# Daniel-Liu-c0deb0t/block-aligner

Hardware: AMD Instinct MI355X
Metric: GCUPS (DP cells/s) on 10 kbp DNA X-drop batch; bit-exact score+CIGAR vs AVX2 (higher is better)
Workload: dtype i16 (saturating lane scores) + i32 block offsets

## Files before the change

block_aligner_amd/csrc/ba_driver.hpp:

```cpp
#pragma once
#include "ba_device.hpp"

namespace ba {

#ifndef BA_BIG
#define BA_BIG 0
#endif
constexpr bool kBig = BA_BIG != 0;
__device__ __forceinline__ void lds_sync() {
    if (kBig) __builtin_amdgcn_fence(__ATOMIC_ACQ_REL, "workgroup");
    else __builtin_amdgcn_fence(__ATOMIC_ACQ_REL, "wavefront");
    __builtin_amdgcn_wave_barrier();
}
__device__ __forceinline__ void lds_fill0(short* a, uint32_t n) {
    for (uint32_t k = 2 * lane_id(); k < n; k += 128) *(int*)(a + k) = 0;
    lds_sync();
}
__device__ __forceinline__ void lds_copy(short* dst, const short* src, uint32_t n) {
    lds_sync();
    for (uint32_t k = 2 * lane_id(); k < n; k += 128) {
        const int v = *(const int*)(src + k);
        lds_sync();
        *(int*)(dst + k) = v;
    }
    lds_sync();
}
__device__ __forceinline__ int lds_prefix_max8(const short* a) {
    lds_sync();
    const int* p = (const int*)a;
    const s16x2 m = as_s(vmax(vmax(p[0], p[1]), vmax(p[2], p[3])));
    return uni(max((int)m.x, (int)m.y));
}
__device__ __forceinline__ int lds_suffix_max2(const short* a, uint32_t n) {
    lds_sync();
    s16x2 m = as_s(*(const int*)(a + n - 2));
    return uni(max((int)m.x, (int)m.y));
}
__device__ __forceinline__ int lds_shift_and_offset(uint32_t n, short* b1, short* b2, const short* t1, const short* t2, int off_add) {
    const int oa = splat(off_add);
    lds_sync();
    const int corner = uni((int)as_s(adds(splat((int)b1[STEP - 1]), oa)).x);
    for (uint32_t base = 0; base < n; base += 128) {
        const uint32_t k = base + 2 * lane_id();
        int v1 = 0, v2 = 0;
        const bool in = k < n;
        if (in) {
            if (k + STEP < n) {
                v1 = adds(*(const int*)(b1 + k + STEP), oa);
                v2 = adds(*(const int*)(b2 + k + STEP), oa);
            } else {
                v1 = *(const int*)(t1 + (k + STEP - n));
                v2 = *(const int*)(t2 + (k + STEP - n));
            }
        }
        lds_sync();
        if (in) { *(int*)(b1 + k) = v1; *(int*)(b2 + k) = v2; }
        lds_sync();
    }
    return corner;
}

struct Move { uint32_t op, di, dj, next; };
constexpr uint32_t TB_PENDING = 3;
__device__ __forceinline__ Move tb_lut(bool right_blk, uint32_t t, uint32_t t2, uint32_t table) {
    constexpr uint32_t OP_M = 1, OP_I = 4, OP_D = 5;
    const uint32_t gapA_op = right_blk ? OP_D : OP_I, gapB_op = right_blk ? OP_I : OP_D;
    const uint32_t A_di = right_blk ? 0 : 1, A_dj = right_blk ? 1 : 0;
    const uint32_t A_tab = right_blk ? 1 : 2, B_tab = right_blk ? 2 : 1;
    if (table == A_tab) return (t2 & 1) ? Move{gapA_op, A_di, A_dj, 0} : Move{gapA_op, A_di, A_dj, A_tab};
    if (table == B_tab) return Move{gapB_op, 1 - A_di, 1 - A_dj, TB_PENDING};
    if (t == 0) return Move{OP_M, 1, 1, 0};
    if (t & 1) return (t2 & 1) ? Move{gapA_op, A_di, A_dj, 0} : Move{gapA_op, A_di, A_dj, A_tab};
    return Move{gapB_op, 1 - A_di, 1 - A_dj, TB_PENDING};
}
__device__ __forceinline__ uint32_t tb_resolve(bool right_blk, uint32_t table, uint32_t nib) {
    return table == TB_PENDING ? ((nib & 8u) ? 0u : (right_blk ? 2u : 1u)) : table;
}
__device__ __forceinline__ uint32_t tb_next(bool right_blk, uint32_t next, uint32_t v) {
    return (next == TB_PENDING && v == 0) ? (right_blk ? 2u : 1u) : next;
}

template <bool RO>
__host__ __device__ constexpr uint32_t slot_cell_byte(uint32_t c) { return RO ? (((c & 2u) << 1) | ((c & 4u) >> 1) | (c & 1u)) : c; }

template <bool RO = false>
__device__ __forceinline__ uint32_t traceback(const BlockRec* __restrict__ blocks, uint32_t nblocks, const uint32_t* __restrict__ trace,
                                     uint32_t i, uint32_t j, const uint8_t* __restrict__ q, const uint8_t* __restrict__ r, uint32_t flags,
                                     uint32_t* __restrict__ out, uint64_t out_lo, uint64_t out_hi, uint32_t* status) {
    const bool eq = flags & F_CIGAR_EQ, local = flags & F_LOCAL, fqs = flags & F_FQS;
    bool stop = false;
    uint64_t wp = out_hi;
    uint32_t run_op = 0, run_len = 0;
    uint32_t table = 0;
    uint32_t bidx = nblocks;
    while ((i > 0 || j > 0) && !stop) {
        BlockRec br;
        for (;;) {
            if (bidx == 0) { *status |= ST_TRACEBACK_LOST; return 0; }
            bidx--;
            br = blocks[bidx];
            if (i >= (br.i & 0x7fffffffu) && j >= br.j) break;
        }
        const bool right_blk = br.trace_base >> 31;
        const bool l2 = br.i >> 31;
        br.i &= 0x7fffffffu;
        if (br.trace_base & 0x40000000u) { *status |= ST_TRACEBACK_LOST; return 0; }
        const uint32_t tbase = br.trace_base & 0x3fffffffu;
        const uint32_t Hv = right_blk ? br.h : br.w;
        const uint32_t nch = Hv > 128 ? Hv / 128 : 1, nl = Hv > 128 ? 64 : Hv / 2;
        while (i >= br.i && j >= br.j && (i > 0 || j > 0)) {
            const uint32_t ci = i - br.i, cj = j - br.j;
            const uint32_t v = right_blk ? ci : cj, w = right_blk ? cj : ci;
            const uint32_t chunk = v >> 7, lane = (v & 127) >> 1;
            if (right_blk && fqs && i == 0) { stop = true; break; }
            uint32_t nib;
            if (l2) {
                const uint32_t cb = slot_cell_byte<RO>(v & 7u);
                const uint32_t word = trace[tbase + (v >> 3) * 8 + (w >> 1) * 2 + (cb >> 2)];
                nib = ((word >> ((cb & 3) * 8 + (w & 1) * 4)) ^ 15u) & 15u;
            } else {
                const uint32_t word = trace[tbase + (((w >> 2) * nch + chunk) * nl + lane) * (local ? 2u : 1u)];
                nib = ((word >> ((v & 1) * 16 + (w & 3) * 4)) ^ 15u) & 15u;
            }
            table = tb_resolve(right_blk, table, nib);
            if (local && table == 0) {
                if (l2) {
                    const uint32_t z = trace[tbase + (uint32_t)br.h * br.w / 8 + (v >> 3) * 2 + ((v >> 2) & 1)];
                    if ((z >> ((v & 3) * 8 + w)) & 1) { stop = true; break; }
                } else {
                    const uint32_t z = trace[tbase + (((w >> 2) * nch + chunk) * nl + lane) * 2u + 1u];
                    if ((z >> ((v & 1) * 16 + (w & 3) * 4)) & 1) { stop = true; break; }
                }
            }
            const Move m = tb_lut(right_blk, nib & 3, (nib >> 2) & 1, table);
            uint32_t op = m.op;
            if (eq && op == 1) op = q[i] == r[j] ? 2 : 3;
            if (m.di > i || m.dj > j) { *status |= ST_TRACEBACK_LOST; return 0; }
            i -= m.di; j -= m.dj; table = tb_next(right_blk, m.next, v);
            if (op == run_op) run_len++;
            else {
                if (run_len) {
                    if (wp == out_lo) { *status |= ST_CIGAR_OVERFLOW; return 0; }
                    out[--wp] = (run_len << 4) | run_op;
                }
                run_op = op; run_len = 1;
            }
        }
    }
    if (run_len) {
        if (wp == out_lo) { *status |= ST_CIGAR_OVERFLOW; return 0; }
        out[--wp] = (run_len << 4) | run_op;
    }
    return (uint32_t)(out_hi - wp);
}

__device__ __forceinline__ uint32_t wave_excl_sum(uint32_t x, uint32_t lane) {
    uint32_t s = x;
#pragma unroll
    for (int d = 1; d < 64; d <<= 1) {
        const uint32_t o = (uint32_t)__shfl_up((int)s, d, 64);
        s += lane >= (uint32_t)d ? o : 0u;
    }
    return s - x;
}
template <bool L2OK, bool RO = false>
__device__ __forceinline__ uint32_t walk_wave(const BlockRec* __restrict__ blocks, uint32_t nblocks_in, const uint32_t* __restrict__ trace,
                                              uint32_t i_in, uint32_t j_in, const uint8_t* __restrict__ q, const uint8_t* __restrict__ r, bool eq,
                                              uint32_t* __restrict__ out, uint64_t out_lo, uint64_t out_hi, uint32_t* status,
                                              uint32_t* __restrict__ lds, uint32_t budget) {
    const uint32_t lane = (uint32_t)lane_id();
    uint32_t lutv0, lutv1;
    {
        const Move a = tb_lut(false, lane & 3, (lane >> 2) & 1, (lane >> 4) & 3), b = tb_lut(true, lane & 3, (lane >> 2) & 1, (lane >> 4) & 3);
        lutv0 = a.op | (a.di << 3) | (a.dj << 4) | (a.next << 5);
        lutv1 = b.op | (b.di << 3) | (b.dj << 4) | (b.next << 5);
    }
    uint32_t i = (uint32_t)uni((int)i_in), j = (uint32_t)uni((int)j_in), bidx = (uint32_t)uni((int)nblocks_in);
    uint32_t table = 0, run_op = 0, run_len = 0, nrun = 0, runbuf = 0, st = 0;
    uint64_t wp = out_hi;
    uint32_t qw0 = 0, rw0 = 0, qwin = 0, rwin = 0;
    auto load_q = [&]() { qw0 = i >= 252u ? (i - 252u) & ~3u : 0u; const uint32_t a = qw0 + 4u * lane; qwin = a <= i ? *(const uint32_t*)(q + a) : 0u; };
    auto load_r = [&]() { rw0 = j >= 252u ? (j - 252u) & ~3u : 0u; const uint32_t a = rw0 + 4u * lane; rwin = a <= j ? *(const uint32_t*)(r + a) : 0u; };
    if (eq) { load_q(); load_r(); }
    auto flush = [&]() {
        if (lane < nrun) out[wp - 1u - lane] = runbuf;
        wp -= nrun; nrun = 0;
    };
    auto emit = [&]() -> bool {
        if (!run_len) return true;
        if (wp - nrun == out_lo) return false;
        asm volatile("s_mov_b32 m0, %2\n\tv_writelane_b32 %0, %1, m0" : "+v"(runbuf) : "s"(__builtin_amdgcn_readfirstlane((int)((run_len << 4) | run_op))), "s"(__builtin_amdgcn_readfirstlane((int)nrun)) : "m0");
        if (++nrun == 64u) flush();
        return true;
    };
    bool ok = true;
    while (ok && (i > 0 || j > 0)) {
        if (bidx == 0) { st = ST_TRACEBACK_LOST; ok = false; break; }
        const uint32_t nvalid = min(bidx, 64u);
        uint4 rec = uint4{0, 0, 0, 0};
        if (lane < nvalid) rec = *(const uint4*)(blocks + (bidx - 1u - lane));
        const bool untr = rec.w & 0x40000000u;
        const uint32_t words = untr ? 0u : (rec.z & 0xffffu) * (rec.z >> 16) / 8u;
        const uint32_t tb = rec.w & 0x3fffffffu;
        uint32_t toff = wave_excl_sum(lane < nvalid ? words : 0u, lane);
        const uint32_t nfit = (uint32_t)__popcll(__ballot(lane < nvalid && toff + words <= budget));
        const uint32_t tb_up = (uint32_t)__shfl_up((int)tb, 1, 64);
        const bool flat = nfit > 1 && !__any(lane > 0 && lane < nfit && tb + words != tb_up);
        if (nfit > 0) {
            const uint32_t total = (uint32_t)__builtin_amdgcn_readlane((int)(toff + words), (int)(nfit - 1u));
            if (flat) {
                const uint32_t lo = (uint32_t)__builtin_amdgcn_readlane((int)tb, (int)(nfit - 1u));
                for (uint32_t x = lane; x < total; x += 64u) lds[x] = trace[lo + x];
                toff = tb - lo;
            } else {
                for (uint32_t k = 0; k < nfit; k++) {
                    const uint32_t base = (uint32_t)__builtin_amdgcn_readlane((int)tb, (int)k), sz = (uint32_t)__builtin_amdgcn_readlane((int)words, (int)k);
                    const uint32_t off = (uint32_t)__builtin_amdgcn_readlane((int)toff, (int)k);
                    for (uint32_t x = lane; x < sz; x += 64u) lds[off + x] = trace[base + x];
                }
            }
            asm volatile("s_waitcnt vmcnt(0) lgkmcnt(0)" ::: "memory");
        }
        const bool direct = nfit == 0;
        const uint32_t ntake = direct ? 1u : nfit;
        auto walk_rects = [&](auto direct_c) {
        constexpr bool DIRECT = decltype(direct_c)::value;
        uint32_t cur = 0;
        while (cur < ntake && ok && (i > 0 || j > 0)) {
            const uint32_t rx = (uint32_t)__builtin_amdgcn_readlane((int)rec.x, (int)cur), bj = (uint32_t)__builtin_amdgcn_readlane((int)rec.y, (int)cur);
            const uint32_t bi = rx & 0x7fffffffu;
            if (!(i >= bi && j >= bj)) { cur++; continue; }
            const uint32_t rz = (uint32_t)__builtin_amdgcn_readlane((int)rec.z, (int)cur), rw = (uint32_t)__builtin_amdgcn_readlane((int)rec.w, (int)cur);
            if (rw & 0x40000000u) { st = ST_TRACEBACK_LOST; ok = false; break; }
            const uint32_t off = DIRECT ? (rw & 0x3fffffffu) : (uint32_t)__builtin_amdgcn_readlane((int)toff, (int)cur);
            const bool right = rw >> 31, l2 = L2OK && (rx >> 31);
            const uint32_t Hv = right ? (rz & 0xffffu) : (rz >> 16);
            const uint32_t nch = Hv > 128u ? Hv / 128u : 1u, nl = Hv > 128u ? 64u : Hv / 2u;
            const uint32_t lutr = right ? lutv1 : lutv0;
            while (i >= bi && j >= bj && (i > 0 || j > 0)) {
                const uint32_t ci = i - bi, cj = j - bj;
                const uint32_t v = right ? ci : cj, w = right ? cj : ci;
                uint32_t widx, sh;
                if (l2) { const uint32_t cb = slot_cell_byte<RO>(v & 7u); widx = (v >> 3) * 8u + (w >> 1) * 2u + (cb >> 2); sh = (cb & 3u) * 8u + (w & 1u) * 4u; }
                else { widx = ((w >> 2) * nch + (v >> 7)) * nl + ((v & 127u) >> 1); sh = (v & 1u) * 16u + (w & 3u) * 4u; }
                uint32_t word;
                if (table == 0u && i > 0u && j > 0u && min(v, w) >= 1u) {
                    const uint32_t lim = min(min(v, w), min(i, j) - 1u);
                    const bool valid = lane <= lim;
                    const uint32_t vv = v - lane, ww = w - lane;
                    uint32_t widx_k, sh_k;
                    if (l2) { const uint32_t cb = slot_cell_byte<RO>(vv & 7u); widx_k = (vv >> 3) * 8u + (ww >> 1) * 2u + (cb >> 2); sh_k = (cb & 3u) * 8u + (ww & 1u) * 4u; }
                    else { widx_k = ((ww >> 2) * nch + (vv >> 7)) * nl + ((vv & 127u) >> 1); sh_k = (vv & 1u) * 16u + (ww & 3u) * 4u; }
                    uint32_t word_k = 0;
                    if (valid) { if constexpr (DIRECT) word_k = trace[off + widx_k]; else word_k = lds[off + widx_k]; }
                    const unsigned long long cm = __ballot(valid && ((word_k >> sh_k) & 3u) == 3u);
                    uint32_t n = cm == ~0ull ? 64u : (uint32_t)__builtin_ctzll(~cm);
                    if (eq && n >= 2u) {
                        if (i < qw0) load_q();
                        if (j < rw0) load_r();
                        n = min(n, min(i - qw0, j - rw0) + 1u);
                    }
                    if (n >= 2u) {
                        bool fits = true;
                        if (!eq) {
                            if (run_op == 1u) run_len += n;
                            else { fits = emit(); run_op = 1u; run_len = n; }
                        } else {
                            const uint32_t qa = i - lane - qw0, ra = j - lane - rw0;
                            const uint32_t qd = (uint32_t)__builtin_amdgcn_ds_bpermute((int)(qa & ~3u), (int)qwin), rd = (uint32_t)__builtin_amdgcn_ds_bpermute((int)(ra & ~3u), (int)rwin);
                            const bool same = ((qd >> ((qa & 3u) * 8u)) & 255u) == ((rd >> ((ra & 3u) * 8u)) & 255u);
                            unsigned long long bits = __ballot(lane < n && same);
                            uint32_t rem = n;
                            while (rem && fits) {
                                const bool e = bits & 1ull;
                                const unsigned long long x = e ? ~bits : bits;
                                const uint32_t len = min(x ? (uint32_t)__builtin_ctzll(x) : 64u, rem), op2 = e ? 2u : 3u;
                                if (op2 == run_op) run_len += len;
                                else { fits = emit(); run_op = op2; run_len = len; }
                                bits = len < 64u ? bits >> len : 0ull; rem -= len;
                            }
                        }
                        if (!fits) { st = ST_CIGAR_OVERFLOW; ok = false; break; }
                        i -= n; j -= n;
                        continue;
                    }
                    word = (uint32_t)__builtin_amdgcn_readlane((int)word_k, 0);
                } else {
                if constexpr (DIRECT) word = (uint32_t)uni((int)trace[off + widx]); else word = (uint32_t)uni((int)lds[off + widx]);
                }
                const uint32_t nib = ((word >> sh) ^ 15u) & 15u;
                table = tb_resolve(right, table, nib);
                const uint32_t m = (uint32_t)__builtin_amdgcn_readlane((int)lutr, (int)((table << 4) | nib));
                uint32_t op = m & 7u;
                const uint32_t di = (m >> 3) & 1u, dj = (m >> 4) & 1u;
                if (eq && op == 1u) {
                    if (i < qw0) load_q();
                    if (j < rw0) load_r();
                    const uint32_t qd = (uint32_t)__builtin_amdgcn_readlane((int)qwin, (int)((i - qw0) >> 2)), rd = (uint32_t)__builtin_amdgcn_readlane((int)rwin, (int)((j - rw0) >> 2));
                    op = ((qd >> ((i & 3u) * 8u)) & 255u) == ((rd >> ((j & 3u) * 8u)) & 255u) ? 2u : 3u;
                }
                if (di > i || dj > j) { st = ST_TRACEBACK_LOST; ok = false; break; }
                i -= di; j -= dj; table = tb_next(right, m >> 5, v);
                if (op == run_op) run_len++;
                else {
                    if (!emit()) { st = ST_CIGAR_OVERFLOW; ok = false; break; }
                    run_op = op; run_len = 1;
                }
            }
        }
        };
        if (direct) walk_rects(std::true_type{}); else walk_rects(std::false_type{});
        bidx -= ntake;
    }
    if (ok && !emit()) { st = ST_CIGAR_OVERFLOW; ok = false; }
    if (!ok) { *status |= st; return 0; }
    flush();
    return (uint32_t)(out_hi - wp);
}

#define BA_RLX_AGENT __ATOMIC_RELAXED, __HIP_MEMORY_SCOPE_AGENT

struct TbLane {
    uint32_t slot, pair, i, j, table, bidx, run_op, run_len, status;
    uint64_t wp, lo;
    const BlockRec* blocks; const uint32_t* trace; const uint8_t* q; const uint8_t* r;
    uint32_t bi, bj, tbase, zoff, nch, nl; bool right, in_rect, l2;
    uint4 nrec[4]; uint32_t nq;
    uint32_t tw_chunk, tw_g, tw_lane0; bool tw_ok;
    uint32_t qw0, rw0;
    uint32_t pv[6], po[6], pmask;
};

__device__ __forceinline__ void tb_emit(TbLane& t, uint32_t* __restrict__ out) {
    if (t.run_len) {
        if (t.wp == t.lo) { t.status |= ST_CIGAR_OVERFLOW; t.i = t.j = 0; return; }
        out[--t.wp] = (t.run_len << 4) | t.run_op;
    }
}
__device__ __forceinline__ void tb_fail(TbLane& t) { t.status |= ST_TRACEBACK_LOST; t.i = t.j = 0; t.run_len = 0; }

constexpr int TB_CELLS_PER_STEP = 4;
#ifndef BA_WALK_CELLS
#define BA_WALK_CELLS 8
#endif
#ifndef BA_RING_DEPTH
#define BA_RING_DEPTH 2
#endif
#ifndef BA_WALK_DEPTH
#define BA_WALK_DEPTH 4
#endif
#ifndef BA_HELPER_CELLS
#define BA_HELPER_CELLS 4
#endif
template <int CELLS = TB_CELLS_PER_STEP, int DEPTH = 1, int LB = (int)TB_LANE_BYTES, bool RO = false>
__device__ __forceinline__ void tb_step(TbLane& t, uint32_t flags, uint32_t* __restrict__ out, unsigned char* lrec,
                                        const unsigned char* lut, unsigned long long* tacc = nullptr) {
    constexpr bool LOCREC = LB == (int)TB_LANE_BYTES_LOC;
    constexpr bool L2OK = LB == (int)TB_LANE_BYTES_L2 || LOCREC;
    constexpr int SEQ_Q = LOCREC ? 80 : (L2OK ? 64 : 40), SEQ_R = SEQ_Q + 16;
    const bool eq = flags & F_CIGAR_EQ, local = LOCREC && (flags & F_LOCAL), fqs = flags & F_FQS;
    BA_TSTAMP(ts0);
    if (!t.in_rect || !(t.i >= t.bi && t.j >= t.bj)) {
        bool found = false, untraced = false;
#pragma unroll
        for (int a = 0; a < DEPTH; a++) {
            if (!found && (a == 0 || t.nq)) {
                if (t.bidx == 0) { tb_fail(t); return; }
                uint4 rec;
                if (t.nq) {
                    rec = t.nrec[0];
#pragma unroll
                    for (int k = 0; k + 1 < DEPTH; k++) t.nrec[k] = t.nrec[k + 1];
                    t.nq--;
                } else rec = *(const uint4*)(t.blocks + t.bidx - 1);
                t.bidx--;
                t.l2 = L2OK && (rec.x >> 31); t.bi = rec.x & 0x7fffffffu; t.bj = rec.y;
                const uint32_t h = rec.z & 0xffffu, w = rec.z >> 16;
                t.in_rect = t.i >= t.bi && t.j >= t.bj;
                t.zoff = h * w / 8;
                t.right = rec.w >> 31;
                t.tbase = rec.w & 0x3fffffffu;
                const uint32_t Hv = t.right ? h : w;
                t.nch = Hv > 128 ? Hv / 128 : 1; t.nl = Hv > 128 ? 64 : Hv / 2;
                untraced = rec.w & 0x40000000u;
                found = t.in_rect;
            }
        }
        if (t.nq == 0 && t.bidx > 0) {
#pragma unroll
            for (int k = 0; k < DEPTH; k++) if (t.bidx > (uint32_t)k) t.nrec[k] = *(const uint4*)(t.blocks + t.bidx - 1 - k);
            t.nq = min((uint32_t)DEPTH, t.bidx);
        }
        t.tw_ok = false;
        if (!t.in_rect) return;
        if (untraced) { tb_fail(t); return; }
    }
    {
        const uint32_t ci = t.i - t.bi, cj = t.j - t.bj;
        const uint32_t v = t.right ? ci : cj, w = t.right ? cj : ci;
        const uint32_t chunk = v >> 7, lc = (v & 127) >> 1, g = w >> 2;
        if (L2OK && t.l2) {
            const uint32_t L8 = v >> 3;
            if (!(t.tw_ok && t.tw_chunk == 0xffffu && L8 - t.tw_lane0 < 2u)) {
                t.tw_chunk = 0xffffu; t.tw_g = 0; t.tw_lane0 = L8 ? L8 - 1 : 0u; t.tw_ok = true;
                const uint32_t* wp = t.trace + t.tbase + t.tw_lane0 * 8;
                uint4 a0, a1, a2, a3;
                __builtin_memcpy(&a0, wp, 16); __builtin_memcpy(&a1, wp + 4, 16); __builtin_memcpy(&a2, wp + 8, 16); __builtin_memcpy(&a3, wp + 12, 16);
                uint4* lw = (uint4*)lrec;
                lw[0] = a0; lw[1] = a1; lw[2] = a2; lw[3] = a3;
                if (local) {
                    uint4 z;
                    __builtin_memcpy(&z, t.trace + t.tbase + t.zoff + t.tw_lane0 * 2, 16);
                    lw[4] = z;
                }
            }
        } else
        if (local) {
            if (!(t.tw_ok && chunk == t.tw_chunk && t.tw_g - g < 2u && lc - t.tw_lane0 < 5u)) {
                t.tw_chunk = chunk; t.tw_g = g; t.tw_lane0 = min(lc >= 4 ? lc - 4 : 0u, t.nl - 5u); t.tw_ok = true;
                const uint32_t* hi = t.trace + t.tbase + ((g * t.nch + chunk) * t.nl + t.tw_lane0) * 2u;
                const uint32_t* lo = g ? hi - t.nch * t.nl * 2u : hi;
                uint4 h0, h1, l0, l1; uint2 h2, l2;
                __builtin_memcpy(&h0, hi, 16); __builtin_memcpy(&h1, hi + 4, 16); __builtin_memcpy(&h2, hi + 8, 8);
                __builtin_memcpy(&l0, lo, 16); __builtin_memcpy(&l1, lo + 4, 16); __builtin_memcpy(&l2, lo + 8, 8);
                uint32_t* lw = (uint32_t*)lrec;
                lw[0] = h0.x; lw[1] = h0.y; lw[2] = h0.z; lw[3] = h0.w; lw[4] = h1.x; lw[5] = h1.y; lw[6] = h1.z; lw[7] = h1.w; lw[8] = h2.x; lw[9] = h2.y;
                lw[10] = l0.x; lw[11] = l0.y; lw[12] = l0.z; lw[13] = l0.w; lw[14] = l1.x; lw[15] = l1.y; lw[16] = l1.z; lw[17] = l1.w; lw[18] = l2.x; lw[19] = l2.y;
            }
        } else
        if (!(t.tw_ok && chunk == t.tw_chunk && t.tw_g - g < 2u && lc - t.tw_lane0 < 5u)) {
            t.tw_chunk = chunk; t.tw_g = g; t.tw_lane0 = min(lc >= 4 ? lc - 4 : 0u, t.nl - 5u); t.tw_ok = true;
            const uint32_t* hi = t.trace + t.tbase + (g * t.nch + chunk) * t.nl + t.tw_lane0;
            const uint32_t* lo = g ? hi - t.nch * t.nl : hi;
            uint32_t wv[10];
            {
                uint4 h4, l4;
                __builtin_memcpy(&h4, hi, 16); __builtin_memcpy(&l4, lo, 16);
                wv[0] = h4.x; wv[1] = h4.y; wv[2] = h4.z; wv[3] = h4.w; wv[4] = hi[4];
                wv[5] = l4.x; wv[6] = l4.y; wv[7] = l4.z; wv[8] = l4.w; wv[9] = lo[4];
            }
#pragma unroll
            for (int k = 0; k < 10; k++) ((uint32_t*)lrec)[k] = wv[k];
        }
        if (eq) {
            if (t.qw0 == 0xffffffffu || t.i < t.qw0 + 8 || t.i >= t.qw0 + 16) {
                t.qw0 = t.i >= 12 ? (t.i - 12) & ~3u : 0;
                const uint32_t* p = (const uint32_t*)(t.q + t.qw0);
                uint32_t b4[4];
#pragma unroll
                for (int k = 0; k < 4; k++) b4[k] = p[k];
#pragma unroll
                for (int k = 0; k < 4; k++) ((uint32_t*)lrec)[SEQ_Q / 4 + k] = b4[k];
            }
            if (t.rw0 == 0xffffffffu || t.j < t.rw0 + 8 || t.j >= t.rw0 + 16) {
                t.rw0 = t.j >= 12 ? (t.j - 12) & ~3u : 0;
                const uint32_t* p = (const uint32_t*)(t.r + t.rw0);
                uint32_t b4[4];
#pragma unroll
                for (int k = 0; k < 4; k++) b4[k] = p[k];
#pragma unroll
                for (int k = 0; k < 4; k++) ((uint32_t*)lrec)[SEQ_R / 4 + k] = b4[k];
            }
        }
    }
#ifdef BA_TIMING
    const unsigned long long ts1 = __builtin_amdgcn_s_memtime();
    asm volatile("s_waitcnt vmcnt(0)" ::: "memory");
    const unsigned long long ts2 = __builtin_amdgcn_s_memtime();
    if (tacc) { tacc[0] += ts1 - ts0; tacc[1] += ts2 - ts1; }
#endif
    {
        bool alive = true;
#pragma unroll
        for (int s = 0; s < CELLS; s++) {
            alive = alive && (t.i > 0 || t.j > 0) && t.i >= t.bi && t.j >= t.bj;
            const uint32_t ci = t.i - t.bi, cj = t.j - t.bj;
            const uint32_t v = t.right ? ci : cj, w = t.right ? cj : ci;
            const uint32_t lc = (v & 127) >> 1;
            if (fqs) {
                const bool stop = alive && t.right && t.i == 0;
                if (stop) t.i = t.j = 0;
                alive = alive && !stop;
            }
            const uint32_t gi = t.tw_g - (w >> 2);
            uint32_t baddr, zaddr = 0, zbit = 0;
            if (L2OK && t.l2) {
                const uint32_t k8 = (v >> 3) - t.tw_lane0;
                alive = alive && t.tw_chunk == 0xffffu && k8 <= 1u;
                baddr = k8 * 32 + (w >> 1) * 8 + slot_cell_byte<RO>(v & 7u);
                zaddr = 64 + k8 * 8 + ((v >> 2) & 1) * 4 + (v & 3); zbit = w;
            } else {
                const uint32_t k = lc - t.tw_lane0;
                alive = alive && (v >> 7) == t.tw_chunk && gi <= 1u && k <= 4u;
                baddr = local ? gi * 40 + k * 8 + (v & 1) * 2 + ((w & 3) >> 1) : gi * 20 + k * 4 + (v & 1) * 2 + ((w & 3) >> 1);
                zaddr = baddr + 4; zbit = (w & 1) * 4;
            }
            const uint32_t qo = t.i - t.qw0, ro = t.j - t.rw0;
            const uint32_t byte = lrec[alive ? baddr : 0u];
            const uint32_t qb = lrec[SEQ_Q + (qo & 15u)], rb = lrec[SEQ_R + (ro & 15u)];
            const uint32_t nib = ((byte >> ((w & 1) * 4)) ^ 15u) & 15u;
            const uint32_t table = tb_resolve(t.right, t.table, nib);
            if (local) {
                const uint32_t zb = lrec[alive ? zaddr : 0u];
                const bool stop = alive && table == 0 && ((zb >> zbit) & 1u);
                if (stop) t.i = t.j = 0;
                alive = alive && !stop;
            }
            const uint32_t m = lut[((uint32_t)t.right << 6) | (table << 4) | nib];
            uint32_t op = m & 7u;
            const uint32_t di = (m >> 3) & 1u, dj = (m >> 4) & 1u;
            const bool is_match = eq && op == 1;
            alive = alive && !(is_match && (qo > 15u || ro > 15u));
            if (is_match) op = qb == rb ? 2u : 3u;
            if (alive && (di > t.i || dj > t.j)) { tb_fail(t); alive = false; }
            const bool same = op == t.run_op;
            if (alive && !same && t.run_len) {
                if (t.wp == t.lo) { t.status |= ST_CIGAR_OVERFLOW; t.i = t.j = 0; alive = false; }
                else out[--t.wp] = (t.run_len << 4) | t.run_op;
            }
            t.i -= alive ? di : 0u; t.j -= alive ? dj : 0u;
            t.table = alive ? tb_next(t.right, m >> 5, v) : t.table;
            t.run_len = alive ? (same ? t.run_len + 1 : 1u) : t.run_len;
            t.run_op = alive ? op : t.run_op;
        }
    }
}

#ifndef BA_TB_FAST
#define BA_TB_FAST 1
#endif
#ifndef BA_TB_FCELLS
#define BA_TB_FCELLS 1
#endif
#ifndef BA_TB_DIAG_RUNS
#define BA_TB_DIAG_RUNS 2
#endif
#ifndef BA_TB_DIAG2
#define BA_TB_DIAG2 1
#endif
#ifndef BA_TB_FDEPTH
#define BA_TB_FDEPTH 3
#endif
typedef uint32_t tb_u32x4 __attribute__((ext_vector_type(4)));
__device__ __forceinline__ uint4 tb_ld16(const void* p) {
    typedef tb_u32x4 __attribute__((aligned(4))) V;
    const tb_u32x4 v = *(const V*)p;
    return uint4{v.x, v.y, v.z, v.w};
}
__device__ __forceinline__ uint32_t ffbl_u32(uint32_t x) { uint32_t r; asm("v_ffbl_b32 %0, %1" : "=v"(r) : "v"(x)); return r; }
__device__ __forceinline__ void tb_prefetch2(TbLane& t) {
    if (t.bidx > 0u) t.nrec[0] = *(const uint4*)(t.blocks + t.bidx - 1);
    if (t.bidx > 1u) t.nrec[1] = *(const uint4*)(t.blocks + t.bidx - 2);
    t.nq = min(2u, t.bidx);
}
template <bool L2W, bool RO = false>
__device__ __forceinline__ void tb_diag_lut_fill(unsigned char* dlut) {
    if constexpr (L2W) {
#pragma unroll
        for (int e = 0; e < 3; e++) {
            const uint32_t idx = (uint32_t)lane_id() + 64u * e;
            const uint32_t k = idx & 7u, p = idx >> 3;
            const uint32_t x = (p - k) & 15u, c = ((p - 16u) - k) & 7u;
            dlut[idx] = (unsigned char)(p < 16u ? (((x & 8u) << 2) | slot_cell_byte<RO>(x & 7u)) : ((c >> 1) << 3));
        }
    }
    {
        const uint32_t idx = (uint32_t)lane_id(), k = idx & 7u, x = ((idx >> 3) - k) & 7u;
        dlut[(L2W ? TB_DIAG_LUT_L2 - TB_DIAG_LUT_STD : 0u) + idx] = (unsigned char)((x < 4u ? 20u : 0u) + ((x & 3u) >> 1));
    }
}
template <int S>
__device__ __forceinline__ void tb_push(TbLane& t, const bool cond, const uint32_t val, bool& ovf) {
    const bool room = t.wp != t.lo, go = cond && room;
    t.wp -= go ? 1u : 0u;
    t.pv[S] = go ? val : t.pv[S];
    t.po[S] = go ? (uint32_t)t.wp - (uint32_t)t.lo : t.po[S];
    t.pmask |= go ? (1u << S) : 0u;
    ovf = ovf || (cond && !room);
}
__device__ __forceinline__ void tb_flush(TbLane& t, uint32_t* __restrict__ out) {
#pragma unroll
    for (int s = 0; s < 6; s++) if ((t.pmask >> s) & 1u) out[t.lo + t.po[s]] = t.pv[s];
    t.pmask = 0;
}

template <bool L2W, int SEQ_Q, int SEQ_R, int S0>
__device__ __forceinline__ void tb_diag(TbLane& t, const bool eq, const unsigned char* lrec, const unsigned char* dlut, bool& ovf) {
    static_assert(BA_TB_DIAG_RUNS >= 1 && BA_TB_DIAG_RUNS <= 2, "two slots per call site");
    const uint32_t ci = t.i - t.bi, cj = t.j - t.bj;
    const uint32_t v = t.right ? ci : cj, w = t.right ? cj : ci;
    bool ok = t.in_rect && t.tw_ok && t.i >= t.bi && t.j >= t.bj && (t.table == 0u || t.table == TB_PENDING);
    uint32_t K = min(min(t.i, t.j), min(v, w) + 1u);
// ... 1461 lines not shown
```

Baseline: 2700.

## Extend traceback diagonal run detection across staged block boundaries and skip redundant probes

In the LDS-staged traceback path, the wave-wide diagonal-match probe can now follow the diagonal across several staged blocks. It builds a per-diagonal-offset owner table in a reserved 64-word LDS slice and uses bpermute to fetch each lane's block record, so a run can jump directly to the block where it ends. A skip counter also suppresses re-probing after a known non-diagonal cell. This is meant to cut the number of serial probe iterations per traceback, at the cost of more per-probe work (prefix max, LDS writes, five bpermutes) and a slightly smaller staging budget.

```diff
diff --git a/block_aligner_amd/csrc/ba_driver.hpp b/block_aligner_amd/csrc/ba_driver.hpp
--- a/block_aligner_amd/csrc/ba_driver.hpp
+++ b/block_aligner_amd/csrc/ba_driver.hpp
@@ -169,6 +169,8 @@
                                               uint32_t* __restrict__ out, uint64_t out_lo, uint64_t out_hi, uint32_t* status,
                                               uint32_t* __restrict__ lds, uint32_t budget) {
     const uint32_t lane = (uint32_t)lane_id();
+    const uint32_t tbudget = budget - 64u;
+    uint32_t* const own = lds + tbudget;
     uint32_t lutv0, lutv1;
     {
         const Move a = tb_lut(false, lane & 3, (lane >> 2) & 1, (lane >> 4) & 3), b = tb_lut(true, lane & 3, (lane >> 2) & 1, (lane >> 4) & 3);
@@ -201,9 +203,9 @@
         if (lane < nvalid) rec = *(const uint4*)(blocks + (bidx - 1u - lane));
         const bool untr = rec.w & 0x40000000u;
         const uint32_t words = untr ? 0u : (rec.z & 0xffffu) * (rec.z >> 16) / 8u;
-        const uint32_t tb = rec.w & 0x3fffffffu;
+        const uint32_t tb = rec.w & 0x3fffffffu, rbi = rec.x & 0x7fffffffu;
         uint32_t toff = wave_excl_sum(lane < nvalid ? words : 0u, lane);
-        const uint32_t nfit = (uint32_t)__popcll(__ballot(lane < nvalid && toff + words <= budget));
+        const uint32_t nfit = (uint32_t)__popcll(__ballot(lane < nvalid && toff + words <= tbudget));
         const uint32_t tb_up = (uint32_t)__shfl_up((int)tb, 1, 64);
         const bool flat = nfit > 1 && !__any(lane > 0 && lane < nfit && tb + words != tb_up);
         if (nfit > 0) {
@@ -225,7 +227,7 @@
         const uint32_t ntake = direct ? 1u : nfit;
         auto walk_rects = [&](auto direct_c) {
         constexpr bool DIRECT = decltype(direct_c)::value;
-        uint32_t cur = 0;
+        uint32_t cur = 0, skip = 0;
         while (cur < ntake && ok && (i > 0 || j > 0)) {
             const uint32_t rx = (uint32_t)__builtin_amdgcn_readlane((int)rec.x, (int)cur), bj = (uint32_t)__builtin_amdgcn_readlane((int)rec.y, (int)cur);
             const uint32_t bi = rx & 0x7fffffffu;
@@ -244,22 +246,52 @@
                 if (l2) { const uint32_t cb = slot_cell_byte<RO>(v & 7u); widx = (v >> 3) * 8u + (w >> 1) * 2u + (cb >> 2); sh = (cb & 3u) * 8u + (w & 1u) * 4u; }
                 else { widx = ((w >> 2) * nch + (v >> 7)) * nl + ((v & 127u) >> 1); sh = (v & 1u) * 16u + (w & 3u) * 4u; }
                 uint32_t word;
-                if (table == 0u && i > 0u && j > 0u && min(v, w) >= 1u) {
-                    const uint32_t lim = min(min(v, w), min(i, j) - 1u);
-                    const bool valid = lane <= lim;
-                    const uint32_t vv = v - lane, ww = w - lane;
-                    uint32_t widx_k, sh_k;
-                    if (l2) { const uint32_t cb = slot_cell_byte<RO>(vv & 7u); widx_k = (vv >> 3) * 8u + (ww >> 1) * 2u + (cb >> 2); sh_k = (cb & 3u) * 8u + (ww & 1u) * 4u; }
-                    else { widx_k = ((ww >> 2) * nch + (vv >> 7)) * nl + ((vv & 127u) >> 1); sh_k = (vv & 1u) * 16u + (ww & 3u) * 4u; }
-                    uint32_t word_k = 0;
-                    if (valid) { if constexpr (DIRECT) word_k = trace[off + widx_k]; else word_k = lds[off + widx_k]; }
-                    const unsigned long long cm = __ballot(valid && ((word_k >> sh_k) & 3u) == 3u);
+                if (table == 0u && skip == 0u && i > 0u && j > 0u && (!DIRECT || min(v, w) >= 1u)) {
+                    uint32_t word_k = 0, own_k = cur;
+                    unsigned long long cm, vm;
+                    if constexpr (DIRECT) {
+                        const uint32_t lim = min(min(v, w), min(i, j) - 1u);
+                        const bool valid = lane <= lim;
+                        const uint32_t vv = v - lane, ww = w - lane;
+                        uint32_t widx_k, sh_k;
+                        if (l2) { const uint32_t cb = slot_cell_byte<RO>(vv & 7u); widx_k = (vv >> 3) * 8u + (ww >> 1) * 2u + (cb >> 2); sh_k = (cb & 3u) * 8u + (ww & 1u) * 4u; }
+                        else { widx_k = ((ww >> 2) * nch + (vv >> 7)) * nl + ((vv & 127u) >> 1); sh_k = (vv & 1u) * 16u + (ww & 3u) * 4u; }
+                        if (valid) word_k = trace[off + widx_k];
+                        vm = __ballot(valid); cm = __ballot(valid && ((word_k >> sh_k) & 3u) == 3u);
+                    } else {
+                        const uint32_t kcur = min(min(v, w), 63u);
+                        const int K = lane > cur && lane < ntake ? min(min((int)(i - rbi), (int)(j - rec.y)), 63) : (lane == cur ? (int)kcur : -1);
+                        const int pm = wave_prefix_max(K);
+                        const int prev = __builtin_amdgcn_update_dpp(-1, pm, 0x138, 0xf, 0xf, false);
+                        const uint32_t kmax = (uint32_t)__builtin_amdgcn_readlane(pm, 63);
+                        for (int kk = lane == cur ? pm + 1 : prev + 1; __any(kk <= pm); kk++)
+                            if (kk <= pm) own[kk] = lane;
+                        asm volatile("" ::: "memory");
+                        const bool mine = lane <= min(kmax, min(i, j) - 1u);
+                        if (mine && lane > kcur) own_k = own[lane];
+                        const int oa = (int)(own_k << 2);
+                        const uint32_t ox = (uint32_t)__builtin_amdgcn_ds_bpermute(oa, (int)rec.x), oy = (uint32_t)__builtin_amdgcn_ds_bpermute(oa, (int)rec.y);
+                        const uint32_t oz = (uint32_t)__builtin_amdgcn_ds_bpermute(oa, (int)rec.z), ow = (uint32_t)__builtin_amdgcn_ds_bpermute(oa, (int)rec.w);
+                        const uint32_t ot = (uint32_t)__builtin_amdgcn_ds_bpermute(oa, (int)toff);
+                        const bool valid = mine && !(ow & 0x40000000u);
+                        const bool oright = ow >> 31, ol2 = L2OK && (ox >> 31);
+                        const uint32_t oci = i - lane - (ox & 0x7fffffffu), ocj = j - lane - oy;
+                        const uint32_t vv = oright ? oci : ocj, ww = oright ? ocj : oci;
+                        const uint32_t oHv = oright ? (oz & 0xffffu) : (oz >> 16);
+                        const uint32_t onch = oHv > 128u ? oHv / 128u : 1u, onl = oHv > 128u ? 64u : oHv / 2u;
+                        uint32_t widx_k, sh_k;
+                        if (ol2) { const uint32_t cb = slot_cell_byte<RO>(vv & 7u); widx_k = (vv >> 3) * 8u + (ww >> 1) * 2u + (cb >> 2); sh_k = (cb & 3u) * 8u + (ww & 1u) * 4u; }
+                        else { widx_k = ((ww >> 2) * onch + (vv >> 7)) * onl + ((vv & 127u) >> 1); sh_k = (vv & 1u) * 16u + (ww & 3u) * 4u; }
+                        if (valid) word_k = lds[ot + widx_k];
+                        vm = __ballot(valid); cm = __ballot(valid && ((word_k >> sh_k) & 3u) == 3u);
+                    }
                     uint32_t n = cm == ~0ull ? 64u : (uint32_t)__builtin_ctzll(~cm);
                     if (eq && n >= 2u) {
                         if (i < qw0) load_q();
                         if (j < rw0) load_r();
                         n = min(n, min(i - qw0, j - rw0) + 1u);
                     }
+                    const uint32_t known = n < 64u ? (uint32_t)(((vm & ~cm) >> n) & 1ull) : 0u;
                     if (n >= 2u) {
                         bool fits = true;
                         if (!eq) {
@@ -281,13 +313,19 @@
                             }
                         }
                         if (!fits) { st = ST_CIGAR_OVERFLOW; ok = false; break; }
-                        i -= n; j -= n;
+                        i -= n; j -= n; skip = known;
+                        if constexpr (!DIRECT) {
+                            const uint32_t last = (uint32_t)__builtin_amdgcn_readlane((int)own_k, (int)(n - 1u));
+                            if (last != cur) { cur = last; break; }
+                        }
                         continue;
                     }
                     word = (uint32_t)__builtin_amdgcn_readlane((int)word_k, 0);
+                    skip = n + known;
                 } else {
                 if constexpr (DIRECT) word = (uint32_t)uni((int)trace[off + widx]); else word = (uint32_t)uni((int)lds[off + widx]);
                 }
+                if (skip) skip--;
                 const uint32_t nib = ((word >> sh) ^ 15u) & 15u;
                 table = tb_resolve(right, table, nib);
                 const uint32_t m = (uint32_t)__builtin_amdgcn_readlane((int)lutr, (int)((table << 4) | nib));
```

Result: faster. 2735 (median of 6 runs) (+1.3%).
